# aask1357/fastenhancer

Measured on AMD Instinct MI355X. Metric: audio frames/sec (hop=256, 16kHz) FastEnhancer_B, higher is better.
Workload: dtype f32

## Files before the change

fastenhancer_amd/csrc/fe_frame8.hip.h:

```cpp
#pragma once
#include "fe_kernels.hip.h"

namespace fe {

constexpr int kThreads8 = 512;
constexpr int kWaves8 = 8;

template <class S>
struct Wg8 {
    using L = Lds<S>;
    static constexpr bool MDFT = (S::NFFT == 512) || (S::C1 < 128);
    static constexpr bool OK0 = L::STAGED && L::SKIPS_LDS && S::GFLAT && S::KT == 1 && S::LOW == 0 && !S::FRNN && !S::TATT && !S::LN && !S::BIDIR &&
                               S::G8P && S::MTC == 4 && S::MT2 == 2 && MDFT && !L::PERHEAD && S::NFFT == kThreads8 && S::NTPW2 == 1;
    static constexpr int NTA = (S::NTC + 1) / 2, NTB = S::NTC - NTA;
    static constexpr int N2A = (S::NT2 + 1) / 2, N2B = S::NT2 - N2A;
    static constexpr int NPW = ceil_div(ceil_div(Pack<S>::umax(), 256), kWaves8);
    static constexpr int HPT = ceil_div(S::F2 * S::C2, kThreads8);
    static constexpr int SLOT = S::U8_SLOT;
    static constexpr int WB0 = L::NOSTAGE_TOTAL, WB1 = WB0 + 2 * SLOT;
    static constexpr int LDM = 13;
    static constexpr int MXB = L::NOSTAGE_TOTAL + 4 * SLOT, MX_FLOATS = round_up(4 * 16 * LDM + 8, 4), MXF = MXB + 4 * 16 * LDM;
    static constexpr int HST = MXB + MX_FLOATS;
    static constexpr bool HSTASH = (size_t)(HST + S::KB * S::F2 * S::C2) * 4 <= 160 * 1024;
    static constexpr size_t BYTES = (size_t)(HST + (HSTASH ? S::KB * S::F2 * S::C2 : 0)) * 4;
    static constexpr int NPWB = ceil_div(ceil_div(SLOT, 256), kWaves8);
    static constexpr bool PLAN_OK = 2 * SLOT >= Pack<S>::umax() && BYTES <= 160 * 1024 && (S::NU & 1) == 0;
    static constexpr bool OK = OK0 && PLAN_OK;
};

template <class S, int NT, int J0, int KS, int NCOLS, int LDO, bool ACT, class AF, class BF, class BI, class SIDE>
__device__ __forceinline__ void conv8(AF&& af, BF&& bf, BI&& bias, const SIDE& side, float* out, int row0, int mt, int lane, float ap = 0.0f) {
    if constexpr (NT > 0) {
        const int li = lane & 15, lg = lane >> 4;
        f32x4 acc[1][NT];
#pragma unroll
        for (int j = 0; j < NT; ++j) acc[0][j] = bias(J0 + j);
        mma_panel<1, NT, KS, Lds<S>::PDK>(acc, [&](int, int ks) { return af(ks); }, [&](int j, int ks) { return bf(J0 + j, ks); }, side);
        side.commit();
#pragma unroll
        for (int j = 0; j < NT; ++j) {
            const int col = 16 * (J0 + j) + li;
            if (col < NCOLS) {
#pragma unroll
                for (int r = 0; r < 4; ++r) {
                    const int m = 16 * mt + 4 * lg + r;
                    float v = acc[0][j][r];
                    if (ACT) v = act_scaled_f<S::EPA>(v, ap);
                    out[(row0 + m) * LDO + col] = v;
                }
            }
        }
    } else {
        constexpr int NSG = (KS + 3) / 4;
#pragma unroll
        for (int g = 0; g < NSG; ++g) side(g, NSG);
        side.commit();
    }
}
template <class S, int NA, int NB, int KS, int NCOLS, int LDO, bool ACT, class AF, class BF, class BI, class SIDE>
__device__ __forceinline__ void conv8_pair(int wh, AF&& af, BF&& bf, BI&& bias, const SIDE& side, float* out, int row0, int mt, int lane,
                                           float ap = 0.0f) {
    if (wh == 0) conv8<S, NA, 0, KS, NCOLS, LDO, ACT>(af, bf, bias, side, out, row0, mt, lane, ap);
    else conv8<S, NB, NA, KS, NCOLS, LDO, ACT>(af, bf, bias, side, out, row0, mt, lane, ap);
}

template <class S, bool DBG, bool PERSIST, bool SLOT = false, bool HIO = false, bool STRM = false>
__global__ void __launch_bounds__(kThreads8) __attribute__((amdgpu_waves_per_eu(2, 2))) fe_frame8_kernel(typename KernelArgs<SLOT, STRM>::type a_in) {
    static_assert(Wg8<S>::OK, "fe_frame8_kernel: shape outside the 512-thread kernel's plan");
    static_assert(!HIO || (SLOT && !DBG), "host audio: slotted production instantiations only");
    static_assert(!STRM || HIO, "packet audio: the host-audio instantiations only");
    typename KernelArgs<SLOT, STRM>::type a = a_in;
    if constexpr (STRM) a.T = 1;
#ifdef FE_PROBE_HOT
    if constexpr (!DBG) a.dbg = nullptr;
#else
    if constexpr (!DBG) { a.dbg = nullptr; a.clk = nullptr; }
#endif
    FE_CLK(62);
    extern __shared__ __attribute__((aligned(16))) float smem[];
    using L = Lds<S>;
    using W8 = Wg8<S>;
    constexpr int N = S::NFFT, H = S::HOP, OVL = S::OVL, F0 = S::F0, F1 = S::F1;
    constexpr int C1 = S::C1, C2 = S::C2, F2 = S::F2, HD = S::HD;
    constexpr int LDC = S::LDC, LDX = S::LDX, LDG = L::LDGX;
    constexpr int NTH = kThreads8;
#ifndef FE_WG8_PDK
#define FE_WG8_PDK 3
#endif
    constexpr int PDK = FE_WG8_PDK;

    const int tid0 = threadIdx.x;
    const int tid = tid0;
    const int lane = tid & 63;
    const int wave0 = __builtin_amdgcn_readfirstlane(tid >> 6);
    const int wave = wave0;
    float hv = 0.0f;
    auto hop_issue = [&](int bb) {
        if constexpr (STRM) {
            const StreamView v = stream_view<H>(a, bb);
            if (v.hops && tid0 >= OVL) hv = stream_sample(a.wav_in, a.format, v.in_off + (tid0 - OVL));
        } else
        if constexpr (HIO) { if (bb < a.B && tid0 >= OVL) hv = a.wav_in[(size_t)bb * a.in_stride + tid0 - OVL]; }
    };
    hop_issue((int)blockIdx.x);
    const float* __restrict__ wp = a.wp;
    WSrc<true> wb;
    constexpr PackedOffsets o = Pack<S>::v;
    wb.rsrc = __builtin_amdgcn_make_buffer_rsrc(const_cast<float*>(a.wp), 0, o.total * 4, 0x00020000);
    wb.lane4 = lane * 4;
    wb.li4 = (lane & 15) * 4;
    wb.lds = nullptr;
    wb.base = 0;
    wb.k4d = 0;
    float ap = 0.0f;
    if constexpr (S::EPP) ap = wp[o.act_p];

    float* sc = smem + L::SC;
    float* Ebuf = smem + L::E;
    float* W0 = smem + L::W0;
    float* W1 = smem + L::W1;
    float2* tw = reinterpret_cast<float2*>(smem + L::TW);
    constexpr int NPW = W8::NPW;
    DmaJobT<NPW> job;
    job.l = smem + W8::WB0;
    job.rsrc = wb.rsrc;
    job.soff = (o.u_off[0] + wave * 256) * 4;
    job.wave = wave;
    job.lane = lane;
    typename Dft<S>::FwdConst dc;
    float fv = 0.0f, fw = 0.0f;
    {
        const StageSide<NPW, o.u_size[0] / 256, kWaves8> st0{&job};
        st0(0, 1);
        float2 twv = make_float2(0.0f, 0.0f);
        if (tid < N / 2) twv = reinterpret_cast<const float2*>(wp + o.twiddle)[tid];
        DmaJobT<NPW> job1 = job;
        job1.l = smem + W8::WB1;
        job1.soff = (o.u_off[1] + wave * 256) * 4;
        const StageSide<NPW, PERSIST ? 0 : o.u_size[1] / 256, kWaves8> st1{&job1};
        if constexpr (!PERSIST) {
            const int b0 = (int)blockIdx.x;
            if constexpr (SLOT) {
                int s0;
                bool live;
                if constexpr (STRM) {
                    const StreamView v0 = stream_view<H>(a, b0);
                    s0 = v0.slot;
                    live = v0.hops != 0 && (unsigned)s0 < (unsigned)a.capacity;
                } else {
                    s0 = a.slots[b0];
                    live = (unsigned)s0 < (unsigned)a.capacity;
                }
                if constexpr (HIO) fv = (tid < OVL) ? (live ? a.cache_stft[(size_t)s0 * OVL + tid] : 0.0f) : hv;
                else fv = (tid < OVL) ? (live ? a.cache_stft[(size_t)s0 * OVL + tid] : 0.0f) : a.wav_in[(size_t)b0 * a.in_stride + tid - OVL];
            } else {
                fv = (tid < OVL) ? a.cache_stft[(size_t)b0 * OVL + tid] : a.wav_in[(size_t)b0 * a.in_stride + tid - OVL];
            }
            fw = wp[o.window + tid];
            if (wave < 4) Dft<S>::load(dc, wb, o, wave);
            st1(0, 1);
        }
        for (int i = tid; i < 2 * S::LDS_S; i += NTH) smem[L::SC + i] = 0.0f;
        for (int i = tid; i < (S::NL + 1) * 2 * LDC; i += NTH) {
            const int e = i / (2 * LDC), q = i - e * (2 * LDC);
            smem[L::E + e * S::ACT + (q >= LDC ? (F1 + 1) * LDC + (q - LDC) : q)] = 0.0f;
        }
        if (tid < N / 2) tw[tid] = twv;
        if (tid < 8) smem[W8::MXF + tid] = 0.0f;
        st0.commit();
        if constexpr (!PERSIST) {
            st1.commit();
            smem[L::FFT_A + tid] = fv * fw;
        }
    }
    __syncthreads();

    int b = (int)blockIdx.x;
    int fc = 0;
    StreamView sv{-1, 0, 0, 0};
#pragma unroll 1
    do {
        int sb = b;
        int nst = a.B;
        if constexpr (SLOT) {
            static_assert(!DBG, "slotted step: production instantiations only");
            if constexpr (STRM) {
                sv = stream_view<H>(a, b);
                sb = sv.slot;
            } else
            sb = a.slots[b];
            nst = a.capacity;
            if constexpr (STRM) {
                if (sv.hops == 0 || (unsigned)sb >= (unsigned)nst) {
                    if (sv.hops) stream_zero_row(a.wav_out, a.format, sv.out_off, H, tid0, NTH);
                    __builtin_amdgcn_s_waitcnt(0);
                    b += (int)gridDim.x;
                    hop_issue(b);
                    continue;
                }
            } else
            if ((unsigned)sb >= (unsigned)nst) {
                if constexpr (HIO) { if (tid0 < H) __builtin_nontemporal_store(0.0f, a.wav_out + (size_t)b * a.out_stride + tid0); }
                else
                if (tid0 < H) a.wav_out[(size_t)b * a.out_stride + tid0] = 0.0f;
                __builtin_amdgcn_s_waitcnt(0);
                b += (int)gridDim.x;
                hop_issue(b);
                continue;
            }
        }
        int lz = 0, lzv = 0;
        if constexpr (PERSIST) { asm volatile("" : "+s"(lz)); asm volatile("" : "+v"(lzv)); }
        const int wave = wave0 + lz;
        const int tid = tid0 + lzv;
        const int lane = tid & 63;
        const int ws = wave & 3, wh = wave >> 2;
        const int li = lane & 15, lg = lane >> 4;
        float* cst = a.cache_stft + (size_t)sb * OVL;
        float* cis = a.cache_istft + (size_t)sb * OVL;
        const int fpar = (S::NU & 1) ? (fc & 1) : 0;
#define FE8_BEGIN_UNIT(U)                                                                          \
        constexpr int fe_un_ = ((U) + 1 == S::NU) ? 0 : (U) + 1;                                   \
        {                                                                                          \
            const int slot_ = ((U) & 1) ^ fpar;                                                    \
            job.l = smem + (slot_ ? W8::WB0 : W8::WB1);                                            \
            job.soff = (o.u_off[fe_un_] + wave * 256) * 4;                                         \
            wb.lds = smem + (slot_ ? W8::WB1 : W8::WB0);                                           \
            wb.base = o.u_off[(U)];                                                                \
        }                                                                                          \
        const StageSide<NPW, ((!PERSIST && ((U) + 1 == S::NU || (U) == 0)) || (U) == S::U_RFPRE + 1) ? 0 : o.u_size[fe_un_] / 256, kWaves8> stage{&job}
        FE_CLK(0);
        float* q0 = smem + L::FFT_A;
        float* q1 = q0 + N;
        float* q3 = smem + L::FFT_B + N;
        {
            if constexpr (PERSIST) {
                if (wave < 4) Dft<S>::load(dc, wb, o, wave);
                const float* xin = a.wav_in + (size_t)b * a.in_stride;
                if constexpr (HIO) {
                    fv = (tid < OVL) ? cst[tid] : hv;
                    hop_issue(b + (int)gridDim.x);
                } else
                fv = (tid < OVL) ? cst[tid] : xin[tid - OVL];
                fw = wp[o.window + tid];
                q0[tid] = fv * fw;
                __syncthreads();
            }
            if (tid >= H) cst[tid - H] = fv;
            FE_CLK(1);
            float* nyq = a.dbg ? a.dbg + (size_t)b * a.dbg_stride + DebugLayout<S>::offset(0) + 2 * F0 : nullptr;
            if (wave < 4) Dft<S>::template forward<false>(q0, q3, tw, dc, wave, lane, nyq);
            __syncthreads();
            FE_CLK(2);
            const float* Xr = q3;
            const float* Xi = q3 + N / 2;
            if (a.dbg) {
                float* dst = a.dbg + (size_t)b * a.dbg_stride + DebugLayout<S>::offset(0);
                for (int f = tid; f < F0; f += NTH) { dst[2 * f] = Xr[f]; dst[2 * f + 1] = Xi[f]; }
            }
            for (int f = tid; f < F0; f += NTH) {
                const float re = Xr[f], im = Xi[f];
                const float mag = fmaxf(sqrtf(re * re + im * im), 1.0e-5f);
                const float g = pow_f(mag, a.compression - 1.0f);
                sc[2 + f] = re * g;
                sc[S::LDS_S + 2 + f] = im * g;
            }
        }
        __syncthreads();
        if (a.dbg) {
            float* dst = a.dbg + (size_t)b * a.dbg_stride + DebugLayout<S>::offset(1);
            for (int f = tid; f < F0; f += NTH) { dst[2 * f] = sc[2 + f]; dst[2 * f + 1] = sc[S::LDS_S + 2 + f]; }
        }

        FE_CLK(3);
        {
            FE8_BEGIN_UNIT(0);
            conv8_pair<S, W8::NTA, W8::NTB, 4, C1, LDC, true>(
                wh,
                [&](int ks) {
                    const int kk = 4 * ks + lg;
                    const int c = kk & 1, s = (kk >> 1) & 3, tp = kk >> 3;
                    return sc[c * S::LDS_S + 4 * (16 * ws + li + tp) + s];
                },
                [&](int j, int ks) { return wb.at(o.enc_pre_w + (j * 4 + ks) * 64); },
                [&](int j) { return wb.at16x4(o.enc_pre_b + j * 64); }, stage, Ebuf, 1, ws, lane, ap);
        }
        __syncthreads();
        dbg_dump<S, NTH>(a, b, 2, Ebuf + LDC, LDC);

        FE_CLK(4);
        static_for<S::NL>([&](auto l_) {
            constexpr int l = decltype(l_)::value;
            const float* in = Ebuf + l * S::ACT;
            float* out = Ebuf + (l + 1) * S::ACT;
            if (l == 0) FE_CLK(40);
            {
                FE8_BEGIN_UNIT(S::U_ENC + l);
                const float* const t0 = in + (16 * ws + li) * LDC + lg;
                conv8_pair<S, W8::NTA, W8::NTB, 3 * S::KS_C, C1, LDC, true>(
                    wh, [&](int ks) { return t0[(ks / S::KS_C) * LDC + 4 * (ks % S::KS_C)]; },
                    [&](int j, int ks) { return wb.at(o.enc_w[l] + (j * (3 * S::KS_C) + ks) * 64); },
                    [&](int j) { return wb.at16x4(o.enc_b[l] + j * 64); }, stage, out, 1, ws, lane, ap);
            }
            if (l == 0) FE_CLK(42);
            __syncthreads();
            if (l == 0) FE_CLK(43);
            dbg_dump<S, NTH>(a, b, 3 + l, out + LDC, LDC);
        });

        float* Xb = smem + L::X;
        float* Hl = smem + L::HL;
        float* Hs = smem + L::HS;
        float* Gi = smem + L::GI;
        float* Y1 = smem + L::Y1;
        float* Y2 = smem + L::Y2;

        FE_CLK(5);
        constexpr int NTPW3 = S::NTPW3;
        constexpr int HPT = W8::HPT;
        constexpr int K2 = S::KS_2;
        f32x4 xr;
        const int g_rt = wave & 1;
        const int g_t0 = wave < 4 ? 3 * (wave >> 1) : 3 * S::G8_NG;
        const float* const sGx = smem + W8::WB0 + 1 * W8::SLOT;
        const float* const sGh = smem + W8::WB0 + 3 * W8::SLOT;
        const float* const sF = smem + W8::WB0 + 0 * W8::SLOT;
        const float* const sQ = smem + W8::WB0 + 2 * W8::SLOT;
        constexpr int NPWB = W8::NPWB;
        DmaJobT<NPWB> jb1, jb2;
        jb1.rsrc = wb.rsrc; jb1.wave = wave; jb1.lane = lane; jb1.l = smem; jb1.soff = 0;
        jb2 = jb1;
        auto stage_to = [&](DmaJobT<NPWB>& j, int src_floats, int dst_floats) { j.l = smem + dst_floats; j.soff = (src_floats + wave * 256) * 4; };
        constexpr int u8_stride = S::KB > 1 ? o.u8_gx[1] - o.u8_gx[0] : 0;
        using StG = StageSide<NPWB, S::U8_G / 256, kWaves8>;
        using StF = StageSide<NPWB, S::U8_F / 256, kWaves8>;
        using StQ = StageSide<NPWB, S::U8_Q / 256, kWaves8>;
        float pe_r[4];
        auto tok_dst = [&](float* base) {
            const int col = 16 * ws + li;
            return base + (16 * wh + 4 * lg) * LDX + (col < C2 ? col : C2);
        };
        int hs_off[HPT];
#pragma unroll
        for (int q = 0; q < HPT; ++q) {
            const int i = tid + q * NTH, f = i / C2;
            hs_off[q] = i < F2 * C2 ? f * LDX + (i - f * C2) : C2;
        }
        {
            constexpr int KS = F1 / 4;
            const float* Ein = Ebuf + S::NL * S::ACT + LDC;
            FE8_BEGIN_UNIT(S::U_RFPRE);
            stage_to(jb1, o.u8_gx[0], W8::WB0 + 1 * W8::SLOT);
            const StG stg{&jb1};
            f32x4 acc[1][1];
            acc_init_zero<1, 1>(acc);
            const int nt = ws < S::NTC ? ws : S::NTC - 1;
            mma_panel<1, 1, KS, PDK>(
                acc, [&](int, int ks) { return wb.at(o.rfpre_lin + (wh * KS + ks) * 64); },
                [&](int, int ks) { return Ein[(4 * ks + lg) * LDC + 16 * nt + li]; }, side2(stage, stg));
            stage.commit();
            stg.commit();
            const int col = 16 * ws + li;
            if (ws < S::NTC && col < C1 && 16 * wh + 4 * lg < F2) {
#pragma unroll
                for (int r = 0; r < 4; ++r) Y1[(16 * wh + 4 * lg + r) * LDC + col] = acc[0][0][r];
            }
        }
        __syncthreads();
        {
            FE8_BEGIN_UNIT(S::U_RFPRE + 1);
            stage_to(jb1, o.u8_gh[0], W8::WB0 + 3 * W8::SLOT);
            const StG stg{&jb1};
            float hpre[HPT];
            const float* hg0 = a.h + (size_t)sb * (F2 * C2);
#pragma unroll
            for (int q = 0; q < HPT; ++q) { const int i = tid + q * NTH; hpre[q] = hg0[i < F2 * C2 ? i : F2 * C2 - 1]; }
            f32x4 acc[1][1];
            const int nt = ws < S::NT2 ? ws : S::NT2 - 1;
            acc[0][0] = wb.at16x4(o.rfpre_b + nt * 64);
            const float* ya = Y1 + (16 * wh + li) * LDC + lg;
            mma_panel<1, 1, S::KS_C, PDK>(
                acc, [&](int, int ks) { return ya[4 * ks]; },
                [&](int, int ks) { return wb.at(o.rfpre_w + (nt * S::KS_C + ks) * 64); }, stg);
            (void)stage;
            stg.commit();
            xr = acc[0][0];
            float* xd = tok_dst(Xb);
#pragma unroll
            for (int r = 0; r < 4; ++r) xd[r * LDX] = acc[0][0][r];
#pragma unroll
            for (int q = 0; q < HPT; ++q) Hs[hs_off[q]] = hpre[q];
        }
        __syncthreads();
        dbg_dump<S, NTH>(a, b, 3 + S::NL, Xb, LDX);

        FE_CLK(6);
#pragma unroll
        for (int k = 0; k < S::KB; ++k) {
            float* hg = a.h + ((size_t)k * nst + sb) * (F2 * C2);
            const int ub = k * u8_stride;
            if (k == 0) FE_CLK(20);
            {
                stage_to(jb1, o.u8_f1[0] + ub, W8::WB0 + 0 * W8::SLOT);
                stage_to(jb2, o.u8_q[0] + ub, W8::WB0 + 2 * W8::SLOT);
                const StF st1{&jb1};
                const StQ st2{&jb2};
                const auto sideg = side2(st1, st2);
                if (k == 0) {
#pragma unroll
                    for (int r = 0; r < 4; ++r) {
                        const int row = 16 * wh + 4 * lg + r, col = 16 * ws + li;
                        pe_r[r] = wb.gather_g(o.blk_pe + (row < F2 ? row : F2 - 1) * C2 + (col < C2 ? col : C2 - 1));
                    }
                }
                const float* xa = Xb + (16 * g_rt + li) * LDX + lg;
                const float* ha = Hs + (16 * g_rt + li) * LDX + lg;
                const float* wx = sGx + g_t0 * (K2 * 64) + lane;
                const float* wh_ = sGh + g_t0 * (K2 * 64) + lane;
                const float* bx = sGx + S::G8_NT * K2 * 64 + g_t0 * 16 + li;
                const float* bh = sGh + S::G8_NT * K2 * 64 + g_t0 * 16 + li;
                __builtin_amdgcn_sched_barrier(0);
                if (k == 0) FE_CLK(45);
                if (wave < 4) {
                    const int ch = 16 * (wave >> 1) + li;
                    float hprev[4];
#pragma unroll
                    for (int r = 0; r < 4; ++r) hprev[r] = Hs[(16 * g_rt + 4 * lg + r) * LDX + ch];
                    const float b0 = bx[0], b1 = bx[16], b2 = bx[32], b3 = bh[32];
                    f32x4 ar = f32x4{b0, b0, b0, b0}, az = f32x4{b1, b1, b1, b1};
                    f32x4 anx = f32x4{b2, b2, b2, b2}, anh = f32x4{b3, b3, b3, b3};
                    mma_panel_sel<1, 3, 2 * K2, PDK>(
                        [&](int, int j, int ks) -> f32x4& { return j == 0 ? ar : (j == 1 ? az : (ks < K2 ? anx : anh)); },
                        [&](int, int ks) { return ks < K2 ? xa[4 * ks] : ha[4 * (ks - K2)]; },
                        [&](int j, int ks) { return ks < K2 ? wx[(j * K2 + ks) * 64] : wh_[(j * K2 + (ks - K2)) * 64]; }, sideg);
                    __builtin_amdgcn_sched_barrier(0);
                    if (k == 0) FE_CLK(46);
                    float hn[4];
#pragma unroll
                    for (int r = 0; r < 4; ++r) {
                        const float rr = sigmoid_pre(ar[r]);
                        const float zz = sigmoid_pre(az[r]);
                        const float nn = tanh_pre(__builtin_fmaf(rr, anh[r], anx[r]));
                        hn[r] = __builtin_fmaf(zz, hprev[r] - nn, nn);
                    }
                    if (16 * g_rt + 4 * lg < F2) {
#pragma unroll
                        for (int r = 0; r < 4; ++r) {
                            const int row = 16 * g_rt + 4 * lg + r;
                            Hl[row * LDX + ch] = hn[r];
                            if constexpr (W8::HSTASH) smem[W8::HST + k * (F2 * C2) + row * C2 + ch] = hn[r];
                            else hg[row * C2 + ch] = hn[r];
                        }
                    }
                } else {
                    constexpr int R = S::G8_R, LDM = W8::LDM;
                    const bool hhalf = wave >= 6;
                    float* mx = smem + W8::MXB + ((hhalf ? 2 : 0) + g_rt) * (16 * LDM);
                    int* mflag = reinterpret_cast<int*>(smem + W8::MXF) + g_rt;
                    const int seq = fc * S::KB + k + 1;
                    f32x4 s0, s1 = f32x4{0.0f, 0.0f, 0.0f, 0.0f};
                    __builtin_amdgcn_s_setprio(3);
                    if (!hhalf) {
                        const float b0 = bx[0];
                        s0 = f32x4{b0, b0, b0, b0};
                        mma_panel_sel<1, 1, K2, PDK>([&](int, int, int ks) -> f32x4& { return (ks & 1) ? s1 : s0; },
                                                     [&](int, int ks) { return xa[4 * ks]; }, [&](int, int ks) { return wx[ks * 64]; }, sideg);
                    } else {
                        const float b1 = bh[0];
                        s0 = f32x4{b1, b1, b1, b1};
                        mma_panel_sel<1, 1, K2, PDK>([&](int, int, int ks) -> f32x4& { return ((ks + K2) & 1) ? s1 : s0; },
                                                     [&](int, int ks) { return ha[4 * ks]; }, [&](int, int ks) { return wh_[ks * 64]; }, sideg);
                    }
                    s0 += s1;
                    __builtin_amdgcn_sched_barrier(0);
                    if (k == 0) FE_CLK(46);
                    if (li < 3 * R) {
#pragma unroll
                        for (int r = 0; r < 4; ++r) mx[(4 * lg + r) * LDM + li] = s0[r];
                    }
                    if (!hhalf) {
                        __atomic_signal_fence(__ATOMIC_SEQ_CST);
                        __builtin_amdgcn_s_waitcnt(0xc07f);
                        if (lane == 0) __hip_atomic_store(mflag, seq, __ATOMIC_RELAXED, __HIP_MEMORY_SCOPE_WORKGROUP);
                        __atomic_signal_fence(__ATOMIC_SEQ_CST);
                    } else {
                        const int row = lane >> 2, c = lane & 3;
                        static_assert(R == 4, "one (row, channel) per lane: sixteen rows x four channels");
                        const int ch = 16 * S::G8_NG + c;
                        const bool live = 16 * g_rt + row < F2;
                        const float hprev = Hs[(16 * g_rt + row) * LDX + ch];
                        __atomic_signal_fence(__ATOMIC_SEQ_CST);
                        while (__builtin_amdgcn_readfirstlane(__hip_atomic_load(mflag, __ATOMIC_RELAXED, __HIP_MEMORY_SCOPE_WORKGROUP)) < seq) {}
                        __atomic_signal_fence(__ATOMIC_SEQ_CST);
                        const float* mxx = smem + W8::MXB + g_rt * (16 * LDM) + row * LDM + c;
                        const float* mxh = mx + row * LDM + c;
                        const float sxr = mxx[0], sxz = mxx[R], sxn = mxx[2 * R];
                        const float shr = mxh[0], shz = mxh[R], shn = mxh[2 * R];
                        const float rr = sigmoid_pre(sxr + shr);
                        const float zz = sigmoid_pre(sxz + shz);
                        const float nn = tanh_pre(__builtin_fmaf(rr, shn, sxn));
                        const float hn = __builtin_fmaf(zz, hprev - nn, nn);
                        if (live) {
                            Hl[(16 * g_rt + row) * LDX + ch] = hn;
                            if constexpr (W8::HSTASH) smem[W8::HST + k * (F2 * C2) + (16 * g_rt + row) * C2 + ch] = hn;
                            else hg[(16 * g_rt + row) * C2 + ch] = hn;
                        }
                    }
                    __builtin_amdgcn_s_setprio(0);
                }
                st1.commit();
                st2.commit();
            }
            if (k == 0) FE_CLK(47);
            __syncthreads();
            if (k == 0) FE_CLK(21);
            if (k == 0) FE_CLK(22);
            const int ntf = ws < S::NT2 ? ws : S::NT2 - 1;
            {
                stage_to(jb1, o.u8_gx[0] + ub + u8_stride, W8::WB0 + 1 * W8::SLOT);
                const StG stn{&jb1};
                f32x4 acc[1][1];
                const float bj = sF[S::NT2 * K2 * 64 + ntf * 16 + li];
                acc[0][0] = f32x4{bj, bj, bj, bj};
                const float* hla = Hl + (16 * wh + li) * LDX + lg;
                const float* wf = sF + ntf * (K2 * 64) + lane;
                if (k + 1 < S::KB) {
                    mma_panel<1, 1, K2, PDK>(acc, [&](int, int ks) { return hla[4 * ks]; }, [&](int, int ks) { return wf[ks * 64]; }, stn);
                    stn.commit();
                } else
                    mma_panel<1, 1, K2, PDK>(acc, [&](int, int ks) { return hla[4 * ks]; }, [&](int, int ks) { return wf[ks * 64]; }, NoSide{});
                float* xd = tok_dst(Xb);
#pragma unroll
                for (int r = 0; r < 4; ++r) {
                    float v = acc[0][0][r] + xr[r];
                    if (k == 0) v += pe_r[r];
                    xr[r] = v;
                    xd[r * LDX] = v;
                }
            }
            __syncthreads();
            dbg_dump<S, NTH>(a, b, 4 + S::NL + 2 * k, Xb, LDX);
            if (k == 0) FE_CLK(23);
            {
                stage_to(jb1, o.u8_f2[0] + ub, W8::WB0 + 0 * W8::SLOT);
                const StF st1{&jb1};
                f32x4 acc[1][NTPW3];
                acc_init_zero<1, NTPW3>(acc);
                __builtin_amdgcn_sched_barrier(0);
                if (k == 0) FE_CLK(50);
                const float* xa = Xb + (16 * wh + li) * LDX + lg;
                mma_panel<1, NTPW3, K2, PDK>(acc, [&](int, int ks) { return xa[4 * ks]; },
                                             [&](int j, int ks) {
                                                 int nt = ws + 4 * j;
                                                 nt = nt < S::NT3 ? nt : S::NT3 - 1;
                                                 return sQ[(nt * K2 + ks) * 64 + lane];
                                             }, st1);
                st1.commit();
                __builtin_amdgcn_sched_barrier(0);
                if (k == 0) FE_CLK(51);
                float* gdst = Gi + (16 * wh + 4 * lg) * LDG + 16 * ws + li;
#pragma unroll
                for (int j = 0; j < NTPW3; ++j)
                    if (ws + 4 * j < S::NT3) {
#pragma unroll
                        for (int r = 0; r < 4; ++r) gdst[r * LDG + 64 * j] = acc[0][j][r];
                    }
                __builtin_amdgcn_sched_barrier(0);
                if (k == 0) FE_CLK(52);
            }
            __syncthreads();
            if (k == 0) FE_CLK(24);
            attention_head<S, 1, LDG>(Gi, Hl, ws * 3 * HD, ws, wh, 1, lane);
            __syncthreads();
            if (k == 0) FE_CLK(25);
            {
                float hpre[HPT];
                if (k + 1 < S::KB) {
                    const float* hgn = hg + (size_t)nst * (F2 * C2);
#pragma unroll
                    for (int q = 0; q < HPT; ++q) { const int i = tid + q * NTH; hpre[q] = hgn[i < F2 * C2 ? i : F2 * C2 - 1]; }
                }
                f32x4 acc[1][1];
                const float bj = sF[S::NT2 * K2 * 64 + ntf * 16 + li];
                acc[0][0] = f32x4{bj, bj, bj, bj};
                const float* hla = Hl + (16 * wh + li) * LDX + lg;
                const float* wf = sF + ntf * (K2 * 64) + lane;
                if (k + 1 < S::KB) {
                    stage_to(jb1, o.u8_gh[0] + ub + u8_stride, W8::WB0 + 3 * W8::SLOT);
                    const StG stn{&jb1};
                    mma_panel<1, 1, K2, PDK>(acc, [&](int, int ks) { return hla[4 * ks]; }, [&](int, int ks) { return wf[ks * 64]; }, stn);
                    stn.commit();
                } else {
                    stage_to(jb1, o.u_off[S::U_RFPOST], W8::WB1);
                    const StageSide<NPWB, o.u_size[S::U_RFPOST] / 256, kWaves8> stn{&jb1};
                    mma_panel<1, 1, K2, PDK>(acc, [&](int, int ks) { return hla[4 * ks]; }, [&](int, int ks) { return wf[ks * 64]; }, stn);
                    stn.commit();
                }
                if (k + 1 < S::KB) {
#pragma unroll
                    for (int q = 0; q < HPT; ++q) Hs[hs_off[q]] = hpre[q];
                }
                float* xd = tok_dst(Xb);
#pragma unroll
                for (int r = 0; r < 4; ++r) {
                    const float v = acc[0][0][r] + xr[r];
                    xr[r] = v;
                    xd[r * LDX] = v;
                }
            }
            __syncthreads();
            if (k == 0) FE_CLK(26);
            dbg_dump<S, NTH>(a, b, 5 + S::NL + 2 * k, Xb, LDX);
        }

        FE_CLK(7);
        {
            constexpr int KS = F2 / 4;
            FE8_BEGIN_UNIT(S::U_RFPOST);
            conv8_pair<S, W8::N2A, W8::N2B, KS, C2, LDX, false>(
                wh, [&](int ks) { return wb.at(o.rfpost_lin + (ws * KS + ks) * 64); },
                [&](int j, int ks) { return Xb[(4 * ks + lg) * LDX + 16 * j + li]; },
                [&](int) { return f32x4{0.0f, 0.0f, 0.0f, 0.0f}; }, stage, Y2, 0, ws, lane);
        }
        __syncthreads();
        float* const Wx = W1;
        float* const Wy = W0;
        for (int i = tid; i < 2 * LDC; i += NTH) {
            const int r = i / LDC, c = i - r * LDC;
            Wy[(r ? F1 + 1 : 0) * LDC + c] = 0.0f;
        }
        if (a.dbg != nullptr) {
            float* dst = a.dbg + (size_t)b * a.dbg_stride + DebugLayout<S>::offset(4 + S::NL + 2 * S::KB);
            for (int i = tid; i < F1 * C1; i += NTH) {
                const int f = i / C1, n = i - f * C1;
                float v = wp[o.rfpost_b + n];
                for (int kk = 0; kk < C2; ++kk) v += Y2[f * LDX + kk] * wp[o.rfpost_w + n * C2 + kk];
                dst[i] = v;
            }
        }

        FE_CLK(8);
        static_for<S::NL>([&](auto l_) {
            constexpr int l = decltype(l_)::value;
            const float* skip = Ebuf + (S::NL - l) * S::ACT;
            {
                FE8_BEGIN_UNIT(S::U_DEC + l * 2);
                constexpr bool FOLD0 = (l == 0);
                constexpr int K0 = FOLD0 ? S::KS_2 : S::KS_C;
                const float* xa = FOLD0 ? Y2 + (16 * ws + li) * LDX + lg : Wx + (16 * ws + li + 1) * LDC + lg;
                const float* sk = skip + (16 * ws + li + 1) * LDC + lg;
                conv8_pair<S, W8::NTA, W8::NTB, K0 + S::KS_C, C1, LDC, true>(
                    wh, [&](int ks) { return ks < K0 ? xa[4 * ks] : sk[4 * (ks - K0)]; },
                    [&](int j, int ks) { return wb.at(o.dec1_w[l] + (j * (K0 + S::KS_C) + ks) * 64); },
                    [&](int j) { return wb.at16x4(o.dec1_b[l] + j * 64); }, stage, Wy, 1, ws, lane, ap);
            }
            __syncthreads();
            {
                FE8_BEGIN_UNIT(S::U_DEC + l * 2 + 1);
                const float* const t0 = Wy + (16 * ws + li) * LDC + lg;
                conv8_pair<S, W8::NTA, W8::NTB, 3 * S::KS_C, C1, LDC, true>(
                    wh, [&](int ks) { return t0[(ks / S::KS_C) * LDC + 4 * (ks % S::KS_C)]; },
                    [&](int j, int ks) { return wb.at(o.dec3_w[l] + (j * (3 * S::KS_C) + ks) * 64); },
                    [&](int j) { return wb.at16x4(o.dec3_b[l] + j * 64); }, stage, Wx, 1, ws, lane, ap);
            }
            __syncthreads();
            dbg_dump<S, NTH>(a, b, 5 + S::NL + 2 * S::KB + l, Wx + LDC, LDC);
        });

        FE_CLK(9);
        float* PT = smem + L::PT;
        typename Dft<S>::InvConst idc;
        float mb0 = 0.0f, mb1 = 0.0f;
        {
            FE8_BEGIN_UNIT(S::U_POST);
            const float* xa = Wx + (16 * ws + li + 1) * LDC + lg;
            const float* sk = Ebuf + (16 * ws + li + 1) * LDC + lg;
            conv8_pair<S, W8::NTA, W8::NTB, 2 * S::KS_C, C1, LDC, true>(
                wh, [&](int ks) { return ks < S::KS_C ? xa[4 * ks] : sk[4 * (ks - S::KS_C)]; },
                [&](int j, int ks) { return wb.at(o.post1_w + (j * (2 * S::KS_C) + ks) * 64); },
                [&](int j) { return wb.at16x4(o.post1_b + j * 64); }, stage, Wy, 1, ws, lane, ap);
        }
        __syncthreads();
        {
            FE8_BEGIN_UNIT(S::U_POST + 1);
            const float* xa = Wy + (16 * ws + li + 1) * LDC + lg;
            conv8_pair<S, 1, 0, S::KS_C, 16, S::LDP, false>(
                wh, [&](int ks) { return xa[4 * ks]; }, [&](int j, int ks) { return wb.at(o.post_t_w + (j * S::KS_C + ks) * 64); },
                [&](int) { return f32x4{0.0f, 0.0f, 0.0f, 0.0f}; }, stage, PT, 0, ws, lane);
            if (wave < 4) Dft<S>::load(idc, wb, o, wave);
            mb0 = wb.scalar(o.post_t_b);
            mb1 = wb.scalar(o.post_t_b + 1);
        }
        __syncthreads();

        FE_CLK(10);
        {
            const float b0 = mb0, b1 = mb1;
            for (int f = tid; f < F0; f += NTH) {
                const int q = f + 2, j1 = q & 3, i1 = q >> 2;
                float m0 = b0, m1 = b1;
                if (i1 < F1) { m0 += PT[i1 * S::LDP + j1]; m1 += PT[i1 * S::LDP + 8 + j1]; }
                if (i1 >= 1) { m0 += PT[(i1 - 1) * S::LDP + j1 + 4]; m1 += PT[(i1 - 1) * S::LDP + 8 + j1 + 4]; }
                if constexpr (S::EPM != kMaskNone) { m0 = mask_f<S::EPM>(m0); m1 = mask_f<S::EPM>(m1); }
                const float xr_ = sc[2 + f], xi_ = sc[S::LDS_S + 2 + f];
                float yr = xr_ * m0 - xi_ * m1;
                float yi = xr_ * m1 + xi_ * m0;
                if (a.dbg) {
                    float* dst = a.dbg + (size_t)b * a.dbg_stride + DebugLayout<S>::offset(5 + 2 * S::NL + 2 * S::KB);
                    dst[2 * f] = m0; dst[2 * f + 1] = m1;
                }
                const float mag = sqrtf(yr * yr + yi * yi);
                const float g = pow_f(mag, 1.0f / a.compression - 1.0f);
                yr *= g; yi *= g;
                if (a.dbg) {
                    float* dst = a.dbg + (size_t)b * a.dbg_stride + DebugLayout<S>::offset(6 + 2 * S::NL + 2 * S::KB);
                    dst[2 * f] = yr; dst[2 * f + 1] = yi;
                    if (f == 0) { dst[2 * F0] = 0.0f; dst[2 * F0 + 1] = 0.0f; }
                }
                q3[f] = yr;
                q3[N / 2 + f] = yi;
            }
        }
        __syncthreads();

        FE_CLK(11);
        {
            const float ow = wp[o.window_istft + tid];
            const float oc = tid < OVL ? cis[tid] : 0.0f;
            if (wave < 4) Dft<S>::template inverse<WSrc<true>, false>(q3, q0, q1, tw, idc, wb, o, wave, lane);
            __syncthreads();
            FE_CLK(12);
            const int pi = Dft<S>::pidx(tid & (Dft<S>::N1 - 1), tid / Dft<S>::N1);
            const float xo = (q0[pi] + q1[pi]) * ow + oc;
            if constexpr (STRM) {
                if (a.format) {
                    const int qv = pcm16_out(xo);
                    const int pw = pcm16_pair(qv, __shfl_down(qv, 1));
                    const int p1 = __shfl_down(pw, 2), p2 = __shfl_down(pw, 4), p3 = __shfl_down(pw, 6);
                    short* orow = reinterpret_cast<short*>(a.wav_out) + sv.out_off;
                    if (tid < H) {
                        if (H % 8 == 0 && (reinterpret_cast<size_t>(orow) & 15) == 0) {
                            if ((tid & 7) == 0) __builtin_nontemporal_store(i32x4{pw, p1, p2, p3}, reinterpret_cast<i32x4*>(orow + tid));
                        } else {
                            __builtin_nontemporal_store((short)qv, orow + tid);
                        }
                    }
                } else {
                    const float x1 = __shfl_down(xo, 1), x2 = __shfl_down(xo, 2), x3 = __shfl_down(xo, 3);
                    float* orow = a.wav_out + sv.out_off;
                    if (tid < H) {
                        if (H % 4 == 0 && (reinterpret_cast<size_t>(orow) & 15) == 0) {
                            if ((tid & 3) == 0) __builtin_nontemporal_store(f32x4{xo, x1, x2, x3}, reinterpret_cast<f32x4*>(orow + tid));
                        } else {
                            __builtin_nontemporal_store(xo, orow + tid);
                        }
                    }
                }
                if (tid >= H) cis[tid - H] = xo;
            } else
            if constexpr (HIO) {
                const float x1 = __shfl_down(xo, 1), x2 = __shfl_down(xo, 2), x3 = __shfl_down(xo, 3);
                float* orow = a.wav_out + (size_t)b * a.out_stride;
                if (tid < H) {
                    if (H % 4 == 0 && (reinterpret_cast<size_t>(orow) & 15) == 0) {
                        if ((tid & 3) == 0) __builtin_nontemporal_store(f32x4{xo, x1, x2, x3}, reinterpret_cast<f32x4*>(orow + tid));
                    } else {
                        __builtin_nontemporal_store(xo, orow + tid);
                    }
                }
                else cis[tid - H] = xo;
            } else {
            if (tid < H) a.wav_out[(size_t)b * a.out_stride + tid] = xo;
            else cis[tid - H] = xo;
            }
            if constexpr (W8::HSTASH) {
                constexpr int N4 = F2 * C2 / 4;
                static_assert((F2 * C2) % 4 == 0 && W8::HST % 4 == 0, "16-byte state rows");
                const f32x4* hst = reinterpret_cast<const f32x4*>(smem + W8::HST);
#pragma unroll
                for (int k = 0; k < S::KB; ++k) {
                    f32x4* dst = reinterpret_cast<f32x4*>(a.h + ((size_t)k * nst + sb) * (F2 * C2));
                    for (int e = tid; e < N4; e += NTH) dst[e] = hst[k * N4 + e];
                }
            }
            if constexpr (PERSIST) __syncthreads();
        }
        FE_CLK(13);
        b += (int)gridDim.x;
        ++fc;
    } while (PERSIST && b < a.B);
#undef FE8_BEGIN_UNIT
    FE_CLK(63);
}

}
```

Before: 8.305 million.

## Precompute decoder skip-connection GEMM halves during attention in transformer blocks

Splits the decoder and post conv GEMMs into the x segment and the encoder-skip segment. The skip segment, which depends only on encoder activations, is now computed early inside the transformer block loop, interleaved with attention (waves group 0 before, group 1 after, with attention raised to higher priority). Its weights are fetched from global memory into registers and the partial sums are held as accumulators, then used as the starting bias of the later decoder convs. The aim is to fill idle time during attention and shorten the decoder critical path, at the cost of many more live registers and possible occupancy pressure.

```diff
diff --git a/fastenhancer_amd/csrc/fe_frame8.hip.h b/fastenhancer_amd/csrc/fe_frame8.hip.h
--- a/fastenhancer_amd/csrc/fe_frame8.hip.h
+++ b/fastenhancer_amd/csrc/fe_frame8.hip.h
@@ -24,7 +24,17 @@
     static constexpr bool HSTASH = (size_t)(HST + S::KB * S::F2 * S::C2) * 4 <= 160 * 1024;
     static constexpr size_t BYTES = (size_t)(HST + (HSTASH ? S::KB * S::F2 * S::C2 : 0)) * 4;
     static constexpr int NPWB = ceil_div(ceil_div(SLOT, 256), kWaves8);
-    static constexpr bool PLAN_OK = 2 * SLOT >= Pack<S>::umax() && BYTES <= 160 * 1024 && (S::NU & 1) == 0;
+    static constexpr int NSK = S::NL + 1;
+    static constexpr int sk_block(int i) { return i % S::KB; }
+    static constexpr int sk_k0(int i) { return i == 0 ? S::KS_2 : S::KS_C; }
+    static constexpr int sk_kt(int i) { return sk_k0(i) + S::KS_C; }
+    static constexpr int sk_g0(int i) { return sk_k0(i) / 4; }
+    static constexpr int sk_ng(int i) { return sk_kt(i) / 4 - sk_g0(i); }
+    static constexpr int sk_nr(int i) { return sk_kt(i) % 4; }
+    static constexpr int sk_max(int (*f)(int)) { int m = 0; for (int i = 0; i < NSK; ++i) m = f(i) > m ? f(i) : m; return m; }
+    static constexpr int SK_NG = sk_max(sk_ng), SK_NR = sk_max(sk_nr) > 0 ? sk_max(sk_nr) : 1;
+    static constexpr bool SK_OK = NSK <= S::KB && Pack<S>::v.conv_k4_delta != 0;
+    static constexpr bool PLAN_OK = 2 * SLOT >= Pack<S>::umax() && BYTES <= 160 * 1024 && (S::NU & 1) == 0 && SK_OK;
     static constexpr bool OK = OK0 && PLAN_OK;
 };
 
@@ -216,6 +226,12 @@
         const int lane = tid & 63;
         const int ws = wave & 3, wh = wave >> 2;
         const int li = lane & 15, lg = lane >> 4;
+        if constexpr (PERSIST) {
+            wb.lane4 = lane * 4;
+            wb.li4 = li * 4;
+            job.wave = wave;
+            job.lane = lane;
+        }
         float* cst = a.cache_stft + (size_t)sb * OVL;
         float* cis = a.cache_istft + (size_t)sb * OVL;
         const int fpar = (S::NU & 1) ? (fc & 1) : 0;
@@ -395,6 +411,35 @@
         dbg_dump<S, NTH>(a, b, 3 + S::NL, Xb, LDX);
 
         FE_CLK(6);
+        f32x4 sk_acc[W8::NSK][W8::NTA];
+        f32x4 sk_q[W8::NTA][W8::SK_NG];
+        float sk_r[W8::NTA][W8::SK_NR];
+        auto sk_fetch = [&](auto i_, auto nt_, auto j0_) {
+            constexpr int i = decltype(i_)::value, NT = decltype(nt_)::value, J0 = decltype(j0_)::value;
+            constexpr int KT = W8::sk_kt(i), G0 = W8::sk_g0(i), NG = W8::sk_ng(i), NR = W8::sk_nr(i);
+            constexpr int w4 = (i < S::NL ? o.dec1_w[i < S::NL ? i : 0] : o.post1_w) + o.conv_k4_delta;
+            constexpr int bi = i < S::NL ? o.dec1_b[i < S::NL ? i : 0] : o.post1_b;
+#pragma unroll
+            for (int j = 0; j < NT; ++j) {
+#pragma unroll
+                for (int g = 0; g < NG; ++g) sk_q[j][g] = wb.at_gv4(w4 + (J0 + j) * (KT * 64) + (G0 + g) * 256, lane * 16);
+#pragma unroll
+                for (int r = 0; r < NR; ++r) sk_r[j][r] = wb.at_gv(w4 + (J0 + j) * (KT * 64) + (KT - NR + r) * 64, lane * 4);
+                sk_acc[i][j] = wb.at_gv4(bi + (J0 + j) * 64, li * 16);
+            }
+        };
+        auto sk_panel = [&](auto i_, auto nt_) {
+            constexpr int i = decltype(i_)::value, NT = decltype(nt_)::value;
+            constexpr int K0 = W8::sk_k0(i), KT = W8::sk_kt(i), G0 = W8::sk_g0(i), NR = W8::sk_nr(i);
+            const float* sk = Ebuf + (i < S::NL ? S::NL - i : 0) * S::ACT + (16 * ws + li + 1) * LDC + lg;
+            mma_panel_sel<1, NT, S::KS_C, PDK>(
+                [&](int, int j, int) -> f32x4& { return sk_acc[i][j]; }, [&](int, int ks) { return sk[4 * ks]; },
+                [&](int j, int ks) {
+                    const int kk = K0 + ks;
+                    return kk < KT - NR ? sk_q[j][kk / 4 - G0][kk % 4] : sk_r[j][kk - (KT - NR)];
+                }, NoSide{});
+        };
+        auto sk_start = [&](auto i_, int j) { return sk_acc[decltype(i_)::value][j < W8::NTA ? j : j - W8::NTA]; };
 #pragma unroll
         for (int k = 0; k < S::KB; ++k) {
             float* hg = a.h + ((size_t)k * nst + sb) * (F2 * C2);
@@ -544,6 +589,12 @@
             {
                 stage_to(jb1, o.u8_f2[0] + ub, W8::WB0 + 0 * W8::SLOT);
                 const StF st1{&jb1};
+                static_for<W8::NSK>([&](auto i_) {
+                    if (W8::sk_block(decltype(i_)::value) == k) {
+                        if (wh == 0) sk_fetch(i_, std::integral_constant<int, W8::NTA>{}, std::integral_constant<int, 0>{});
+                        else sk_fetch(i_, std::integral_constant<int, W8::NTB>{}, std::integral_constant<int, W8::NTA>{});
+                    }
+                });
                 f32x4 acc[1][NTPW3];
                 acc_init_zero<1, NTPW3>(acc);
                 __builtin_amdgcn_sched_barrier(0);
@@ -570,7 +621,19 @@
             }
             __syncthreads();
             if (k == 0) FE_CLK(24);
+            auto sk_host = [&]() {
+                static_for<W8::NSK>([&](auto i_) {
+                    if (W8::sk_block(decltype(i_)::value) == k) {
+                        if (wh == 0) sk_panel(i_, std::integral_constant<int, W8::NTA>{});
+                        else if constexpr (W8::NTB > 0) sk_panel(i_, std::integral_constant<int, W8::NTB>{});
+                    }
+                });
+            };
+            if (wh == 0) sk_host();
+            __builtin_amdgcn_s_setprio(1);
             attention_head<S, 1, LDG>(Gi, Hl, ws * 3 * HD, ws, wh, 1, lane);
+            __builtin_amdgcn_s_setprio(0);
+            if (wh != 0) sk_host();
             __syncthreads();
             if (k == 0) FE_CLK(25);
             {
@@ -642,17 +705,16 @@
         FE_CLK(8);
         static_for<S::NL>([&](auto l_) {
             constexpr int l = decltype(l_)::value;
-            const float* skip = Ebuf + (S::NL - l) * S::ACT;
             {
                 FE8_BEGIN_UNIT(S::U_DEC + l * 2);
                 constexpr bool FOLD0 = (l == 0);
                 constexpr int K0 = FOLD0 ? S::KS_2 : S::KS_C;
                 const float* xa = FOLD0 ? Y2 + (16 * ws + li) * LDX + lg : Wx + (16 * ws + li + 1) * LDC + lg;
-                const float* sk = skip + (16 * ws + li + 1) * LDC + lg;
-                conv8_pair<S, W8::NTA, W8::NTB, K0 + S::KS_C, C1, LDC, true>(
-                    wh, [&](int ks) { return ks < K0 ? xa[4 * ks] : sk[4 * (ks - K0)]; },
+                static_assert(K0 == W8::sk_k0(l), "the x segment comes first");
+                conv8_pair<S, W8::NTA, W8::NTB, K0, C1, LDC, true>(
+                    wh, [&](int ks) { return xa[4 * ks]; },
                     [&](int j, int ks) { return wb.at(o.dec1_w[l] + (j * (K0 + S::KS_C) + ks) * 64); },
-                    [&](int j) { return wb.at16x4(o.dec1_b[l] + j * 64); }, stage, Wy, 1, ws, lane, ap);
+                    [&](int j) { return sk_start(l_, j); }, stage, Wy, 1, ws, lane, ap);
             }
             __syncthreads();
             {
@@ -674,11 +736,11 @@
         {
             FE8_BEGIN_UNIT(S::U_POST);
             const float* xa = Wx + (16 * ws + li + 1) * LDC + lg;
-            const float* sk = Ebuf + (16 * ws + li + 1) * LDC + lg;
-            conv8_pair<S, W8::NTA, W8::NTB, 2 * S::KS_C, C1, LDC, true>(
-                wh, [&](int ks) { return ks < S::KS_C ? xa[4 * ks] : sk[4 * (ks - S::KS_C)]; },
+            static_assert(W8::sk_k0(S::NL) == S::KS_C, "the x segment comes first");
+            conv8_pair<S, W8::NTA, W8::NTB, S::KS_C, C1, LDC, true>(
+                wh, [&](int ks) { return xa[4 * ks]; },
                 [&](int j, int ks) { return wb.at(o.post1_w + (j * (2 * S::KS_C) + ks) * 64); },
-                [&](int j) { return wb.at16x4(o.post1_b + j * 64); }, stage, Wy, 1, ws, lane, ap);
+                [&](int j) { return sk_start(std::integral_constant<int, S::NL>{}, j); }, stage, Wy, 1, ws, lane, ap);
         }
         __syncthreads();
         {
```

New measurement: 8.104 million. -2.4%, worse.
